# cdglissov/recurrent-flows-msc

Hardware: AMD Instinct MI355X
Metric: frames/sec, RFN SM-MNIST 64x64 train step (fwd+bwd+Adam) (higher is better)
Workload: dtype f32 (forward convolutions fp32-grade: fused scaled-fp16 split f16x3s / three-piece bf16x6 split; gradient convolutions bf16x3 split MFMA; fp32 accumulate everywhere); 1 GPU; RFN SM-MNIST 64x64 canonical (K=10 L=5 Hd=256 h=200 z=56), global_batch=32, seq_len=20, train step; global_batch=32, seq_len=20, parallelism=dp1

## Files before the change

### include/rfn_hip.h

```cpp
#ifndef RFN_HIP_H
#define RFN_HIP_H

#ifdef __cplusplus
extern "C" {
#endif

typedef void* rfn_stream_t;

int rfn_abi_version(void);
const char* rfn_last_error(void);

int rfn_squeeze2d_f32(const float* x, long x_ns, float* y, long y_ns, int N, int C, int H, int W, int undo,
                      rfn_stream_t stream);

int rfn_channel_stats_f32(const float* x, long x_ns, float* mean, float* var_unbiased, int N, int C, int HW,
                          rfn_stream_t stream);

int rfn_actnorm_invconv_fwd_f32(const float* x, long x_ns, const float* bias, const float* logs, const float* Wm,
                                float* z, long z_ns, int N, int C, int HW, rfn_stream_t stream);
int rfn_actnorm_invconv_bwd_f32(const float* x, long x_ns, const float* bias, const float* logs, const float* Wm,
                                const float* gz, long gz_ns, float* gx, long gx_ns, float* gW, float* gbias,
                                float* glogs, int N, int C, int HW, rfn_stream_t stream);
#define RFN_INVCONV_MAX_STEPS 32
#define RFN_INVCONV_MAX_CHANNELS 96
// ... 77 lines not shown
int rfn_gather_affine_f32(const float* P, const float* o_in, long o_ns, const float* b3, const float* l3, float* o_out,
                          float* z, long z_ns, const float* scale, const float* scale_shift, float* logdet,
                          int clamp_type, int N, int C, int H, int W, rfn_stream_t stream);
int rfn_affine_zeros_bwd_f32(const float* zout, long zout_ns, const float* o, long o_ns, const float* gout, long gout_ns,
                             const float* glogdet, const float* scale, const float* scale_shift, const float* l3,
                             float* gz, long gz_ns, float* gpre, long gpre_ns, float* gscale, float* gscale_shift,
                             float* gb3, float* gl3, int clamp_type, int N, int C, int HW, rfn_stream_t stream);

int rfn_glow_shell_fwd_f32(float* z, long z_ns, const float* P, const float* o_in, long o_ns, const float* b3,
                           const float* l3, float* o_out, const float* scale, const float* scale_shift, float* logdet,
                           int clamp_type, const float* bias, const float* logs, const float* Wm, float* znext,
                           long znext_ns, int ld_const, int N, int C, int H, int W, rfn_stream_t stream);
long rfn_glow_shell_fwd_ld_floats(int N, int C, int H, int W);
int rfn_logdet_reduce_f32(const float* part, int n_launch, float* logdet, int accumulate, int N, int C, int H, int W,
                          rfn_stream_t stream);
const char* rfn_glow_shell_fwd_kernel_label(int N, int C, int H, int W, int head);
const char* rfn_glow_shell_bwd_kernel_label(int N, int C, int HW, int tail);
int rfn_glow_shell_supported(int N, int C, int H, int W);
int rfn_glow_shell_bwd_f32(const float* x, long x_ns, const float* bias, const float* logs, const float* Wm,
                           const float* gz, long gz_ns, float* gW, float* gbias, float* glogs, const float* o, long o_ns,
                           const float* glogdet, const float* scale, const float* scale_shift, const float* l3,
                           float* gz_prev, long gz_prev_ns, float* gpre, long gpre_ns, float* gscale,
                           float* gscale_shift, float* gb3, float* gl3, int clamp_type, int ld_const, int N, int C,
                           int HW, rfn_stream_t stream);
int rfn_actnorm_invconv_bwd_ld_f32(const float* x, long x_ns, const float* bias, const float* logs, const float* Wm,
                                   const float* gz, long gz_ns, float* gx, long gx_ns, float* gW, float* gbias,
                                   float* glogs, const float* glogdet, int N, int C, int HW, rfn_stream_t stream);

int rfn_dgrad_small_supported(int N, int Cin, int Cout, int H, int W);
int rfn_conv3x3_smallcout_bf16x3(const float* in, long in_ns, int Cin, const float* wpk, float* out1, long out1_ns,
                                 float* out2, long out2_ns, int Cout, int cout_split, int acc1, int acc2, int N, int H,
                                 int W, rfn_stream_t stream);

int rfn_gemm_wgrad_bf16x3(const float* a, long a_ns, int M, const float* b, long b_ns, int Nc, float* gw, int F, int HW,
                          rfn_stream_t stream);
int rfn_gemm_wgrad_grouped_bf16x3(const float* const* a, long a_ns, int M, const float* const* b, long b_ns, int Nc,
                                  float* const* gw, int G, int F, int HW, rfn_stream_t stream);
const char* rfn_gemm_wgrad_kernel_label_bf16x3(int M, int Nc, long a_ns, long b_ns, int G, int F, int HW);
int rfn_conv3x3_wgrad_implicit_bf16x3(const float* g, long g_ns, int Cout, const float* in1, long in1_ns, int C1,
                                      const float* in2, long in2_ns, int C2, float* gw, int F, int H, int W,
                                      rfn_stream_t stream);
int rfn_conv3x3_wgrad_implicit_grouped_bf16x3(const float* const* g, long g_ns, int Cout, const float* const* in1,
                                              long in1_ns, int C1, const float* const* in2, long in2_ns, int C2,
                                              float* const* gw, int G, int F, int H, int W, rfn_stream_t stream);
const char* rfn_conv3x3_wgrad_implicit_kernel_label_bf16x3(int Cout, long g_ns, int G, int F, int H, int W);
int rfn_im2col3x3_f32(const float* in1, long in1_ns, int C1, const float* in2, long in2_ns, int C2, float* out, int N,
                      int H, int W, rfn_stream_t stream);

long rfn_packed_weight_size(int Cout, int Cin, int ks);
int rfn_pack_conv_weight_f32(const float* w, float* wpk, int Cout, int Cin, int ks, int transpose_flip,
                             rfn_stream_t stream);

int rfn_conv2d_wgrad_f32(const float* in1, long in1_ns, int C1, const float* in2, long in2_ns, int C2,
                         const float* g, long g_ns, int Cout, float* gwt, int N, int H, int W, int ks,
                         rfn_stream_t stream);
const char* rfn_conv2d_wgrad_kernel_label_f32(int ks, int Cin, int Cout, int H, int W);
int rfn_wgrad_finish_f32(const float* gwt, float* gw, int Cout, int Cin, int ks, int accumulate, rfn_stream_t stream);

int rfn_tap_gather_f32(const float* P, const float* bias, const float* logs, float* o, int N, int C, int H, int W,
                       rfn_stream_t stream);
int rfn_tap_scatter_f32(const float* g, float* Gs, int N, int C, int H, int W, rfn_stream_t stream);

int rfn_conv_epilogue_bwd_f32(const float* y, long y_ns, const float* gy, long gy_ns, float* gu, long gu_ns,
                              const float* logs, float* gb, float* gl, int N, int C, int HW, int ep_mode, int act,
                              rfn_stream_t stream);

// ... 127 lines not shown
```

### recurrent-flows-msc_amd/csrc/conv_bf16x3.hip

```cpp
#include "conv_common.h"

typedef __bf16 bf16x8 __attribute__((ext_vector_type(8)));
typedef unsigned int u32x4 __attribute__((ext_vector_type(4)));

static inline void packed_dims_b3(int Cout_l, int Cin_l, int* CoutP, int* Cin16) {
    *CoutP = ((Cout_l + 255) / 256) * 256;
    *Cin16 = (Cin_l + 15) / 16;
}

extern "C" long rfn_packed_weight_size_bf16x3(int Cout, int Cin, int ks) {
    int a, b, c, d;
    packed_dims_b3(Cout, Cin, &a, &b);
    packed_dims_b3(Cin, Cout, &c, &d);
    long s0 = (long)b * ks * ks * 4 * a * 4, s1 = (long)d * ks * ks * 4 * c * 4;
    return s0 > s1 ? s0 : s1;
}
extern "C" long rfn_packed_weight_size_bf16x6(int Cout, int Cin, int ks) {
    return rfn_packed_weight_size_bf16x3(Cout, Cin, ks) / 2 * 3;
}

struct PackDesc {
    const float* w;
    float* wpk;
    int Cout, Cin, ks, mode;
// ... 355 lines not shown
    constexpr int NPOS = (KS == 1) ? 1 : (BPX >= 256 ? 4 : (BPX >= 128 ? 2 : 1));
    constexpr int P2 = (KS == 1 && BPX < 256) ? (BPX >= 64 ? BPX : 64) : 256;
    if (IMG > P2 * NPOS) {
        rfn_set_error("conv2d(bf16x3): map %dx%d needs %d LDS slots (> %d supported)", p.H, p.W, IMG, P2 * NPOS);
        return -7;
    }
    size_t lds = (size_t)NPL * (KC / 8) * IMG * 16 + (size_t)(KC / 16) * KS * KS * NPL * 2 * BCO * 16 + 4 * BCO * 4;
    auto kern = conv_b3_kernel<KS, WCO, WPX, TCO, TPX, KC, NPL>;
    if (lds > 65536) (void)hipFuncSetAttribute((const void*)kern, hipFuncAttributeMaxDynamicSharedMemorySize, (int)lds);
    dim3 grid(p.n_wtiles * p.n_htiles * p.n_ftiles, ceil_div(p.Cout, BCO));
    p.ksplit = 1;
    const int wgs = grid.x * grid.y;
    const int nchunks = (p.Cin8 * 16 + KC - 1) / KC;
    const int HW = p.H * p.W;
    const bool dense = p.out1_ns == (long)p.cout_split * HW &&
                       (p.cout_split == p.Cout || p.out2_ns == (long)(p.Cout - p.cout_split) * HW);
    if (wgs < 128 && nchunks >= 8 && p.ep_mode != 1 && p.ep_mode != 4 && !p.acc1 && !p.acc2 && dense) {
        int ks_ = 512 / wgs;
        if (ks_ > nchunks / 2) ks_ = nchunks / 2;
        if (ks_ > 1) {
            p.ksplit = ks_;
            p.ws_stride = (long)p.N * p.Cout * HW;
            p.ws = rfn_workspace(s, (size_t)ks_ * (size_t)p.ws_stride);
            if (!p.ws) return -8;
        }
    }
    grid.z = p.ksplit;
    hipLaunchKernelGGL(kern, grid, dim3(256), lds, s, p);
    if (p.ksplit > 1) splitk_reduce(p, s);
    return 0;
}

enum ConvB3Route { G3_32x128, G3_64x64, G3_64x128, G1_32x128, G1_64x64, G1_128x128, G1_256x64, WS1, WS3_ACTBWD, WS3_27,
                   WS3_45 };
static const struct { const char* label; int BPX, WPX; } kConvB3Routes[] = {
    {"conv_b3_kernel<3,1,4,1,1,16>", 128, 4},
    {"conv_b3_kernel<3,2,2,1,1,16>", 64, 2},
    {"conv_b3_kernel<3,2,2,1,2,16>", 128, 2},
    {"conv_b3_kernel<1,1,4,1,1,32>", 128, 4},
    {"conv_b3_kernel<1,2,2,1,1,32>", 64, 2},
    {"conv_b3_kernel<1,2,2,2,2,32>", 128, 2},
    {"conv_b3_kernel<1,4,1,2,2,32>", 64, 1},
    {"conv1x1_ws_kernel<16>", 32, 0},
    {"conv3x3_ws_kernel<1,2,0>", 64, 0},
    {"conv3x3_ws_kernel<3,2,1>", 64, 0},
    {"conv3x3_ws_kernel<5,1,1>", 32, 0},
};
static_assert(sizeof(kConvB3Routes) / sizeof(kConvB3Routes[0]) == WS3_45 + 1, "one row per route");

static ConvB3Route choose_conv_b3(const ConvParams& p, int ks) {
    static const bool ws_off = getenv("RFN_CONV_WS") && atoi(getenv("RFN_CONV_WS")) == 0;
    const int Cin = p.C1 + p.C2, Cout = p.Cout;
    const long npix = (long)p.N * p.H * p.W;
    if (p.npl != 3 && !ws_off && Cout % 256 == 0 && npix >= 64L * 256) {
        if (ks == 1 && p.C2 == 0 && Cin > 128 && Cin <= 256) return WS1;
        const int PT = (p.ep_mode == 4 || Cin <= 24) ? 2 : 1;
        const int TH = 32 * PT / (p.W >= 32 ? 32 : (p.W > 0 ? p.W : 1));
        const bool pow2 = (p.H & (p.H - 1)) == 0 && (p.W & (p.W - 1)) == 0;
        if (ks == 3 && pow2 && p.W >= 8 && (long)p.H * p.W >= 64 && p.H >= TH && p.cout_split == Cout && !p.acc1) {
            if (p.ep_mode == 4 && Cin <= 8 && p.C2 == 0) return WS3_ACTBWD;
            if (p.ep_mode >= 0 && p.ep_mode <= 3 && Cin <= 40) return Cin <= 24 ? WS3_27 : WS3_45;
        }
    }
    const bool few_px = npix * ((Cout + 127) / 128) < 256L * 128;
    if (ks == 3) return Cout <= 32 ? G3_32x128 : (few_px ? G3_64x64 : G3_64x128);
    if (Cout <= 32) return G1_32x128;
    if (few_px || Cout <= 64) return G1_64x64;
    return Cout <= 128 ? G1_128x128 : G1_256x64;
}
static int dispatch_conv_b3(ConvParams& p, int ks, hipStream_t s);

static ConvParams conv_b3_shape(int npl, int C1, int C2, int Cout, int cout_split, int acc1, int ep_mode, int N, int H,
                                int W) {
    ConvParams p;
    memset(&p, 0, sizeof(p));
    p.npl = npl; p.C1 = C1; p.C2 = C2; p.Cout = Cout; p.cout_split = cout_split; p.acc1 = acc1; p.ep_mode = ep_mode;
    p.N = N; p.H = H; p.W = W;
    return p;
}
extern "C" const char* rfn_conv2d_kernel_label_bf16x3(int npl, int ks, int C1, int C2, int Cout, int cout_split, int acc1,
                                                     int ep_mode, int N, int H, int W) {
    return kConvB3Routes[choose_conv_b3(conv_b3_shape(npl, C1, C2, Cout, cout_split, acc1, ep_mode, N, H, W), ks)].label;
}
extern "C" int rfn_conv2d_dgrad_act_rows_bf16x3(int N, int H, int W, int ks, int Cout, int Cin) {
    const auto& r = kConvB3Routes[choose_conv_b3(conv_b3_shape(2, Cin, 0, Cout, Cout, 0, 4, N, H, W), ks)];
    if (r.WPX == 0) {
// ... 359 lines not shown
static int launch_conv1x1_ws(ConvParams& p, hipStream_t s) {
    const int HW = p.H * p.W;
    const long total = (long)p.N * HW;
    const int n_tiles = (int)((total + 31) / 32);
    int hw_shift = -1;
    if ((HW & (HW - 1)) == 0) hw_shift = ilog2(HW);
    p.ksplit = 1;
    const size_t lds = (size_t)2 * 2 * 32 * 32 * 16 + 4 * 256 * 4;
    auto kern = conv1x1_ws_kernel<16>;
    (void)hipFuncSetAttribute((const void*)kern, hipFuncAttributeMaxDynamicSharedMemorySize, (int)lds);
    dim3 grid(n_tiles < 256 ? n_tiles : 256, p.Cout / 256);
    hipLaunchKernelGGL(kern, grid, dim3(512), lds, s, p, n_tiles, hw_shift);
    return 0;
}

template <int KS, int WCO, int WPX, int TCO, int TPX, int KC>
static int launch_conv_b3_npl(ConvParams& p, hipStream_t s) {
    return p.npl == 3 ? launch_conv_b3<KS, WCO, WPX, TCO, TPX, KC, 3>(p, s) : launch_conv_b3<KS, WCO, WPX, TCO, TPX, KC>(p, s);
}

static int dispatch_conv_b3(ConvParams& p, int ks, hipStream_t s) {
    switch (choose_conv_b3(p, ks)) {
        case G3_32x128:  return launch_conv_b3_npl<3, 1, 4, 1, 1, 16>(p, s);
        case G3_64x64:   return launch_conv_b3_npl<3, 2, 2, 1, 1, 16>(p, s);
        case G3_64x128:  return launch_conv_b3_npl<3, 2, 2, 1, 2, 16>(p, s);
        case G1_32x128:  return launch_conv_b3_npl<1, 1, 4, 1, 1, 32>(p, s);
        case G1_64x64:   return launch_conv_b3_npl<1, 2, 2, 1, 1, 32>(p, s);
        case G1_128x128: return launch_conv_b3_npl<1, 2, 2, 2, 2, 32>(p, s);
        case G1_256x64:  return launch_conv_b3_npl<1, 4, 1, 2, 2, 32>(p, s);
        case WS1:        return launch_conv1x1_ws(p, s);
        case WS3_ACTBWD: return launch_conv3x3_ws_t<1, 2, false>(p, s);
        case WS3_27:     return launch_conv3x3_ws_t<3, 2>(p, s);
        case WS3_45:     return launch_conv3x3_ws_t<5, 1>(p, s);
    }
    return -9;
}
```

### recurrent-flows-msc_amd/csrc/conv_common.h

```cpp
#pragma once
#include "common.h"
#include "../../include/rfn_hip.h"
#include <stdlib.h>

typedef float f32x16 __attribute__((ext_vector_type(16)));
typedef float f32x4 __attribute__((ext_vector_type(4)));

struct ConvParams {
    const float* in1;
    const float* in2;
    long in1_ns, in2_ns;
    int C1, C2;
    const float* wpk;
    float* out1;
    float* out2;
    long out1_ns, out2_ns;
    int Cout, cout_split, acc1, acc2;
    int N, H, W;
    int CoutP, Cin8;
    int ep_mode, act;
    const float* p0;
    const float* p1;
    int TWp, TH, TF, tw_shift, th_shift;
    int n_wtiles, n_htiles, n_ftiles;
    int P2, P2_shift;
    int ksplit;
    int w_lds_off;
    const float* ybuf;
    long ybuf_ns;
    int npl;
    float* part;
    float* ws;
    long ws_stride;
};

static __global__ void splitk_reduce_kernel(const float* __restrict__ ws, long stride, int ksplit, float* __restrict__ out1,
                                            long n1, float* __restrict__ out2, long n2) {
    const long n = n1 + n2;
    for (long i = (long)blockIdx.x * blockDim.x + threadIdx.x; i < n; i += (long)gridDim.x * blockDim.x) {
        float a = ws[i];
        for (int z = 1; z < ksplit; ++z) a += ws[(long)z * stride + i];
        if (i < n1) out1[i] = a;
        else out2[i - n1] = a;
    }
}
static inline void splitk_reduce(const ConvParams& p, hipStream_t s) {
    const long HW = (long)p.H * p.W, n1 = (long)p.N * p.cout_split * HW, n2 = (long)p.N * (p.Cout - p.cout_split) * HW;
    long blocks = (n1 + n2 + 255) / 256;
    if (blocks > 2048) blocks = 2048;
    hipLaunchKernelGGL(splitk_reduce_kernel, dim3((unsigned)blocks), dim3(256), 0, s, p.ws, p.ws_stride, p.ksplit, p.out1, n1,
                       p.out2, n2);
}

template <int TCO, int TPX, int BCO, bool FASTONLY = false>
__device__ __forceinline__ void conv_epilogue(const ConvParams& p, f32x16 (&acc)[TCO][TPX], const float* ep,
                                              const int co_base, const int wco, const int kk, const int HW,
                                              const int (&pn)[TPX], const int (&ppix)[TPX],
                                              const bool (&pvalid)[TPX], const int prow = 0,
                                              float* const lds_part = nullptr, const bool lds_shared = false) {
    const int cl_base = wco * (32 * TCO) + 4 * kk;
    const bool fast = FASTONLY || ((co_base + 32 * TCO <= p.Cout) && (p.cout_split == p.Cout));
    if (!FASTONLY && p.ep_mode == 4) {
        if (co_base + 32 * TCO > p.Cout) return;
        const float* ybase[TPX];
        float* obase[TPX];
#pragma unroll
        for (int t = 0; t < TPX; ++t) {
            const long off = (long)(co_base + 4 * kk) * HW + ppix[t];
            ybase[t] = pvalid[t] ? p.ybuf + pn[t] * p.ybuf_ns + off : p.ybuf + (long)(co_base + 4 * kk) * HW;
            obase[t] = p.out1 + pn[t] * p.out1_ns + off;
        }
        const int l31 = threadIdx.x & 31;
#pragma unroll
        for (int a = 0; a < TCO; ++a) {
            float yv[16][TPX];
#pragma unroll
            for (int r = 0; r < 16; ++r)
#pragma unroll
                for (int t = 0; t < TPX; ++t)
                    yv[r][t] = ybase[t][(long)(a * 32 + (r & 3) + 8 * (r >> 2)) * HW];
#pragma unroll
            for (int r = 0; r < 16; ++r) {
                const int cidx = a * 32 + (r & 3) + 8 * (r >> 2);
                const float e1 = ep[BCO + cl_base + cidx];
                float sb = 0.f, sl = 0.f;
#pragma unroll
                for (int t = 0; t < TPX; ++t) {
// ... 9 lines not shown
                }
                sb = half_wave_sum_dpp(sb);
                sl = half_wave_sum_dpp(sl);
                if (l31 == 16) {
                    if (lds_part && lds_shared) {
                        float* dst = lds_part + (cl_base + cidx) * 2;
                        atomicAdd(dst, sb);
                        atomicAdd(dst + 1, sl);
                    } else if (lds_part) {
                        float* dst = lds_part + (cl_base + cidx) * 2;
                        dst[0] += sb;
                        dst[1] += sl;
                    } else {
                        float* dst = p.part + co_base + cidx + 4 * kk;
                        atomicAdd(dst, sb);
                        atomicAdd(dst + p.Cout, sl);
                    }
                }
            }
        }
        return;
    }
    if (fast) {
        float* obase[TPX];
        float* const o1 = (!FASTONLY && p.ksplit > 1) ? p.ws + (long)blockIdx.z * p.ws_stride : p.out1;
#pragma unroll
        for (int t = 0; t < TPX; ++t)
            obase[t] = o1 + pn[t] * p.out1_ns + (long)(co_base + 4 * kk) * HW + ppix[t];
#pragma unroll
        for (int a = 0; a < TCO; ++a) {
#pragma unroll
            for (int r = 0; r < 16; ++r) {
                const int cidx = a * 32 + (r & 3) + 8 * (r >> 2);
                float e0 = 0.f, e1 = 1.f;
                if (p.ep_mode != 0) {
                    e0 = blockIdx.z == 0 ? ep[cl_base + cidx] : 0.f;
                    e1 = ep[BCO + cl_base + cidx];
                }
#pragma unroll
                for (int t = 0; t < TPX; ++t) {
                    float v = acc[a][t][r];
                    if (p.ep_mode != 0) v = (v + e0) * e1;
                    if (p.ep_mode == 1) {
                        if (p.act == 1) v = v > 0.f ? v : 0.f;
                        if (p.act == 2) v = v > 0.f ? v : 0.2f * v;
                    }
                    if (pvalid[t]) {
                        float* dst = obase[t] + (long)cidx * HW;
                        if (FASTONLY || p.ksplit > 1) {
                            *dst = v;
                        } else {
                            if (p.acc1) v += *dst;
                            *dst = v;
                        }
                    }
                }
            }
        }
        return;
    }
    if (FASTONLY) return;
#pragma unroll
    for (int a = 0; a < TCO; ++a) {
#pragma unroll
        for (int r = 0; r < 16; ++r) {
            const int cidx = a * 32 + (r & 3) + 8 * (r >> 2);
// ... 12 lines not shown
            const int oc = first ? co : co - p.cout_split;
            const int accm = first ? p.acc1 : p.acc2;
#pragma unroll
            for (int t = 0; t < TPX; ++t) {
                if (!pvalid[t]) continue;
                float v = acc[a][t][r];
                if (p.ep_mode != 0) v = (v + e0) * e1;
                if (p.ep_mode == 1) {
                    if (p.act == 1) v = v > 0.f ? v : 0.f;
                    if (p.act == 2) v = v > 0.f ? v : 0.2f * v;
                }
                float* dst = obase + pn[t] * ons + (long)oc * HW + ppix[t];
                if (p.ksplit > 1) {
                    *dst = v;
                } else {
                    if (accm) v += *dst;
                    *dst = v;
                }
            }
        }
    }
}

static inline void tile_geometry(int H, int W, int BPX, int* TWp, int* TH, int* TF) {
    int tw = next_pow2(W);
    if (tw > 32) tw = 32;
    if (tw > BPX) tw = BPX;
    int th = next_pow2(H);
    if (th > BPX / tw) th = BPX / tw;
    *TWp = tw;
    *TH = th;
    *TF = BPX / (tw * th);
}
```

### recurrent-flows-msc_amd/rfn_hip/lib.py

```python
import ctypes
import os

import torch

_HERE = os.path.dirname(os.path.abspath(__file__))
LIB_PATH = os.path.join(_HERE, "librfn_hip.so")

_c_f = ctypes.c_void_p
_c_i = ctypes.c_int
_c_l = ctypes.c_long
_c_s = ctypes.c_void_p

SIGNATURES = {
    "rfn_abi_version": [],
    "rfn_last_error": [],
    "rfn_squeeze2d_f32": [_c_f, _c_l, _c_f, _c_l, _c_i, _c_i, _c_i, _c_i, _c_i, _c_s],
    "rfn_channel_stats_f32": [_c_f, _c_l, _c_f, _c_f, _c_i, _c_i, _c_i, _c_s],
    "rfn_actnorm_invconv_fwd_f32": [_c_f, _c_l, _c_f, _c_f, _c_f, _c_f, _c_l, _c_i, _c_i, _c_i, _c_s],
    "rfn_actnorm_invconv_bwd_f32": [_c_f, _c_l, _c_f, _c_f, _c_f, _c_f, _c_l, _c_f, _c_l, _c_f, _c_f, _c_f,
                                    _c_i, _c_i, _c_i, _c_s],
    "rfn_invconv_weights_fwd_f32": [ctypes.c_void_p] * 5 + [_c_f, _c_f, _c_i, _c_i, _c_i, _c_s],
    "rfn_invconv_weights_bwd_f32": [ctypes.c_void_p] * 5 + [_c_f, _c_f, _c_f, _c_f, _c_f, _c_i, _c_i, _c_i, _c_s],
    "rfn_invconv_actnorm_rev_f32": [_c_f, _c_l, _c_f, _c_f, _c_f, _c_f, _c_l, _c_i, _c_i, _c_i, _c_s],
    "rfn_conv2d_fwd_f32": [_c_f, _c_l, _c_i, _c_f, _c_l, _c_i, _c_f, _c_f, _c_l, _c_f, _c_l, _c_i, _c_i, _c_i, _c_i,
                           _c_i, _c_i, _c_i, _c_i, _c_i, _c_f, _c_f, _c_i, _c_s],
    "rfn_conv2d_kernel_label_f32": [_c_i] * 5,
    "rfn_conv2d_fwd_bf16x3": [_c_f, _c_l, _c_i, _c_f, _c_l, _c_i, _c_f, _c_f, _c_l, _c_f, _c_l, _c_i, _c_i, _c_i, _c_i,
                              _c_i, _c_i, _c_i, _c_i, _c_i, _c_f, _c_f, _c_i, _c_s],
    "rfn_packed_weight_size_bf16x3": [_c_i, _c_i, _c_i],
    "rfn_pack_conv_weight_bf16x3": [_c_f, _c_f, _c_i, _c_i, _c_i, _c_i, _c_s],
    "rfn_packed_weight_size_bf16x6": [_c_i, _c_i, _c_i],
    "rfn_pack_conv_weight_bf16x6": [_c_f, _c_f, _c_i, _c_i, _c_i, _c_i, _c_s],
    "rfn_conv2d_fwd_bf16x6": [_c_f, _c_l, _c_i, _c_f, _c_l, _c_i, _c_f, _c_f, _c_l, _c_f, _c_l, _c_i, _c_i, _c_i, _c_i,
                              _c_i, _c_i, _c_i, _c_i, _c_i, _c_f, _c_f, _c_i, _c_s],
    "rfn_conv2d_kernel_label_bf16x3": [_c_i] * 11,
    "rfn_conv2d_dgrad_act_rows_bf16x3": [_c_i, _c_i, _c_i, _c_i, _c_i, _c_i],
    "rfn_conv2d_dgrad_act_bf16x3": [_c_f, _c_l, _c_i, _c_f, _c_f, _c_l, _c_f, _c_i, _c_f, _c_l, _c_f, _c_i, _c_i, _c_i,
                                    _c_i, _c_i, _c_s],
    "rfn_gather_affine_f32": [_c_f, _c_f, _c_l, _c_f, _c_f, _c_f, _c_f, _c_l, _c_f, _c_f, _c_f, _c_i, _c_i, _c_i, _c_i,
                              _c_i, _c_s],
    "rfn_affine_zeros_bwd_f32": [_c_f, _c_l, _c_f, _c_l, _c_f, _c_l, _c_f, _c_f, _c_f, _c_f, _c_f, _c_l, _c_f, _c_l, _c_f,
                                 _c_f, _c_f, _c_f, _c_i, _c_i, _c_i, _c_i, _c_s],
    "rfn_glow_shell_fwd_f32": [_c_f, _c_l, _c_f, _c_f, _c_l, _c_f, _c_f, _c_f, _c_f, _c_f, _c_f, _c_i, _c_f, _c_f, _c_f,
                               _c_f, _c_l, _c_i, _c_i, _c_i, _c_i, _c_i, _c_s],
    "rfn_glow_shell_bwd_f32": [_c_f, _c_l, _c_f, _c_f, _c_f, _c_f, _c_l, _c_f, _c_f, _c_f, _c_f, _c_l, _c_f, _c_f, _c_f,
                               _c_f, _c_f, _c_l, _c_f, _c_l, _c_f, _c_f, _c_f, _c_f, _c_i, _c_i, _c_i, _c_i, _c_i, _c_s],
    "rfn_actnorm_invconv_bwd_ld_f32": [_c_f, _c_l, _c_f, _c_f, _c_f, _c_f, _c_l, _c_f, _c_l, _c_f, _c_f, _c_f, _c_f, _c_i,
                                       _c_i, _c_i, _c_s],
    "rfn_dgrad_small_supported": [_c_i, _c_i, _c_i, _c_i, _c_i],
    "rfn_conv3x3_smallcout_bf16x3": [_c_f, _c_l, _c_i, _c_f, _c_f, _c_l, _c_f, _c_l, _c_i, _c_i, _c_i, _c_i, _c_i, _c_i,
                                     _c_i, _c_s],
    "rfn_gemm_wgrad_grouped_bf16x3": [_c_f, _c_l, _c_i, _c_f, _c_l, _c_i, _c_f, _c_i, _c_i, _c_i, _c_s],
    "rfn_conv3x3_wgrad_implicit_grouped_bf16x3": [_c_f, _c_l, _c_i, _c_f, _c_l, _c_i, _c_f, _c_l, _c_i, _c_f, _c_i, _c_i,
                                                  _c_i, _c_i, _c_s],
    "rfn_coupling_po_supported": [_c_i, _c_i, _c_i, _c_i, _c_i, _c_i],
    "rfn_coupling_po_packed_bytes": [_c_i, _c_i],
    "rfn_coupling_po_pack": [_c_f, _c_i, _c_s],
    "rfn_coupling_po_fwd": [_c_f, _c_l, _c_f, _c_l, _c_f, _c_f, _c_f, _c_f, _c_f, _c_f, _c_l, _c_f, _c_l, _c_f, _c_l,
                            _c_f, _c_f, _c_i, _c_i, _c_i, _c_i, _c_i, _c_i, _c_s],
    "rfn_glow_shell_fwd_ld_floats": [_c_i, _c_i, _c_i, _c_i],
    "rfn_logdet_reduce_f32": [_c_f, _c_i, _c_f, _c_i, _c_i, _c_i, _c_i, _c_i, _c_s],
    "rfn_glow_shell_fwd_kernel_label": [_c_i] * 5,
    "rfn_glow_shell_bwd_kernel_label": [_c_i] * 4,
    "rfn_glow_shell_supported": [_c_i] * 4,
    "rfn_coupling_po_mask_floats": [_c_i, _c_i, _c_i],
    "rfn_coupling_po_bwd_supported": [_c_i, _c_i, _c_i, _c_i],
    "rfn_coupling_po_bwd_packed_bytes": [_c_i],
    "rfn_coupling_po_pack_bwd": [_c_f, _c_i, _c_s],
    "rfn_coupling_po_bwd_part_floats": [_c_i, _c_i, _c_i],
    "rfn_coupling_po_bwd": [_c_f, _c_l, _c_f, _c_f, _c_f, _c_f, _c_f, _c_f, _c_l, _c_f, _c_l, _c_f, _c_i, _c_i, _c_i, _c_i,
                            _c_i, _c_s],
    "rfn_coupling_po_bwd_finish": [ctypes.c_void_p] * 8 + [_c_i, _c_i, _c_i, _c_s],
    "rfn_gemm_wgrad_bf16x3": [_c_f, _c_l, _c_i, _c_f, _c_l, _c_i, _c_f, _c_i, _c_i, _c_s],
    "rfn_conv3x3_wgrad_implicit_bf16x3": [_c_f, _c_l, _c_i, _c_f, _c_l, _c_i, _c_f, _c_l, _c_i, _c_f, _c_i, _c_i, _c_i,
                                          _c_s],
    "rfn_gemm_wgrad_kernel_label_bf16x3": [_c_i, _c_i, _c_l, _c_l, _c_i, _c_i, _c_i],
    "rfn_conv3x3_wgrad_implicit_kernel_label_bf16x3": [_c_i, _c_l, _c_i, _c_i, _c_i, _c_i],
    "rfn_im2col3x3_f32": [_c_f, _c_l, _c_i, _c_f, _c_l, _c_i, _c_f, _c_i, _c_i, _c_i, _c_s],
    "rfn_packed_weight_size": [_c_i, _c_i, _c_i],
    "rfn_pack_conv_weight_f32": [_c_f, _c_f, _c_i, _c_i, _c_i, _c_i, _c_s],
    "rfn_conv2d_wgrad_f32": [_c_f, _c_l, _c_i, _c_f, _c_l, _c_i, _c_f, _c_l, _c_i, _c_f, _c_i, _c_i, _c_i, _c_i, _c_s],
    "rfn_conv2d_wgrad_kernel_label_f32": [_c_i] * 5,
    "rfn_wgrad_finish_f32": [_c_f, _c_f, _c_i, _c_i, _c_i, _c_i, _c_s],
    "rfn_tap_gather_f32": [_c_f, _c_f, _c_f, _c_f, _c_i, _c_i, _c_i, _c_i, _c_s],
# ... 145 lines not shown
```

### recurrent-flows-msc_amd/rfn_hip/ops.py

```python
import collections
import ctypes
import functools

import torch

from . import lib as L

_i = ctypes.c_int
_l = ctypes.c_long

import os

CONV_PRECISION = os.environ.get("RFN_CONV_PRECISION", "mixed")


def bwd_b3():
    return CONV_PRECISION in ("bf16x3", "mixed")


MIXED_FWD = os.environ.get("RFN_MIXED_FWD", "bf16x6")


def fwd_prec(H, W):
    if CONV_PRECISION == "mixed":
# ... 309 lines not shown
            assert t[4].numel() == 65536 and t[5].numel() == 65536 and t[2].is_contiguous() and t[5].is_contiguous()
        L.call("rfn_coupling_po_bwd_finish", *cols, _i(len(tk)), _i(nblk), _i(K1),
               meta=_shell("po_bwd_finish", tk[0][7], len(tk) * (nblk * 512 + 512 * K1 + 131072 + 1024) / 1024.0))


def conv2d_raw(in1, in2, wpk, Cout, ks, ep_mode=0, p0=None, p1=None, act=0, out1=None, out2=None, cout_split=None,
               acc1=False, acc2=False, prec=None):
    N, C1, H, W = in1.shape
    C2 = 0 if in2 is None else int(in2.shape[1])
    i1p, i1ns = L.frames(in1, "in1")
    i2p, i2ns = (None, 0) if in2 is None else L.frames(in2, "in2")
    if cout_split is None:
        cout_split = Cout
    if out1 is None:
        out1 = torch.empty((N, cout_split, H, W), device=in1.device, dtype=torch.float32)
    o1p, o1ns = L.frames(out1, "out1")
    o2p, o2ns = (None, 0) if out2 is None else L.frames(out2, "out2")
    prec = prec if prec is not None else ("bf16x3" if bwd_b3() else "f32")
    fn = {"bf16x3": "rfn_conv2d_fwd_bf16x3", "bf16x6": "rfn_conv2d_fwd_bf16x6", "f32": "rfn_conv2d_fwd_f32"}[prec]
    x6 = prec == "bf16x6"
    kname = (kernel_label("rfn_conv2d_kernel_label_f32", ks, Cout, N, H, W) if prec == "f32" else
             kernel_label("rfn_conv2d_kernel_label_bf16x3", 3 if x6 else 2, ks, C1, C2, Cout, cout_split, 1 if acc1 else 0,
                          ep_mode, N, H, W) + (" x6" if x6 else ""))
    L.call(fn, i1p, _l(i1ns), _i(C1), i2p, _l(i2ns), _i(C2),
           L.dev(wpk), o1p, _l(o1ns), o2p,
           _l(o2ns), _i(Cout), _i(cout_split), _i(1 if acc1 else 0), _i(1 if acc2 else 0), _i(N), _i(H), _i(W), _i(ks),
           _i(ep_mode), L.dev(p0), L.dev(p1), _i(act),
           meta=("conv", kname,
                 2.0 * N * H * W * (C1 + C2) * Cout * ks * ks,
                 "N%d %d+%d->%d %dx%d k%d ep%d%s" % (N, C1, C2, Cout, H, W, ks, ep_mode,
                                                  "" if cout_split == Cout else " split"),
                 4.0 * (N * H * W * (C1 + C2 + Cout) + (C1 + C2) * Cout * ks * ks)))
    return out1


def gemm_wgrad(a, b, M, Nc, arena=None):
    F_, HW = int(a.shape[0]), _hw(a)
    ap, ans = L.frames(a, "a")
    bp, bns = L.frames(b, "b")
    gw = _zeros(arena, M, Nc, device=a.device)
    L.call("rfn_gemm_wgrad_bf16x3", ap, _l(ans), _i(M), bp, _l(bns), _i(Nc), L.dev(gw), _i(F_), _i(HW),
           meta=("wgrad", kernel_label("rfn_gemm_wgrad_kernel_label_bf16x3", M, Nc, ans, bns, 0, F_, HW),
                 2.0 * F_ * HW * M * Nc, "F%d %dx%d HW%d" % (F_, M, Nc, HW), 4.0 * (F_ * HW * (M + Nc) + M * Nc)))
    return gw


def conv2d_wgrad_b3(in1, in2, g, Cout, ks, arena=None):
    N, C1, H, W = in1.shape
    C2 = 0 if in2 is None else int(in2.shape[1])
    Cin = C1 + C2
    if ks == 1:
        x = in1 if in2 is None else torch.cat((in1, in2), 1)
        return gemm_wgrad(g, x, Cout, Cin, arena).view(Cout, Cin, 1, 1)
    if Cin <= Cout and W % 8 == 0 and os.environ.get("RFN_WGRAD_IMPLICIT") != "0":
        i1p, i1ns = L.frames(in1, "in1")
        i2p, i2ns = (None, 0) if in2 is None else L.frames(in2, "in2")
        gp, gns = L.frames(g, "g")
        gw = _zeros(arena, Cout, 9 * Cin, device=in1.device)
        L.call("rfn_conv3x3_wgrad_implicit_bf16x3", gp, _l(gns), _i(Cout), i1p, _l(i1ns), _i(C1), i2p, _l(i2ns), _i(C2),
               L.dev(gw), _i(N), _i(H), _i(W),
               meta=("wgrad", kernel_label("rfn_conv3x3_wgrad_implicit_kernel_label_bf16x3", Cout, gns, 0, N, H, W),
                     2.0 * N * H * W * Cout * 9 * Cin, "F%d %dx%d HW%d implicit3x3" % (N, Cout, 9 * Cin, H * W),
                     4.0 * (N * H * W * (Cout + Cin) + Cout * 9 * Cin)))
        return gw.view(Cout, Cin, 3, 3)
    if Cin <= Cout:
        i1p, i1ns = L.frames(in1, "in1")
# ... 1301 lines not shown
```

Before: 11030 frames/s.

## Add persistent register-weight conv3x3 kernel for few-channel convolutions

Adds a new conv3x3 kernel for layers with few input and output channels (at most two 16x32 MFMA tiles). It keeps all weights in registers and runs as a persistent grid over spatial tiles, with a double-buffered LDS halo tile that is split into bf16 planes on the fly. The conv router picks it automatically for qualifying large-pixel convolutions, and an environment variable can turn it off. The aim is to fix poor utilisation and weight-reload overhead of the generic routes on low-channel convolutions, at the cost of heavy register use and one more code path.

```diff
diff --git a/include/rfn_hip.h b/include/rfn_hip.h
--- a/include/rfn_hip.h
+++ b/include/rfn_hip.h
@@ -133,6 +133,12 @@
                                  float* out2, long out2_ns, int Cout, int cout_split, int acc1, int acc2, int N, int H,
                                  int W, rfn_stream_t stream);
 
+int rfn_conv3x3_fewch_supported(int npl, int C1, int C2, int Cout, int H, int W);
+int rfn_conv3x3_fewch_bf16x3(const float* in1, long in1_ns, int C1, const float* in2, long in2_ns, int C2,
+                             const float* wpk, float* out, long out_ns, int Cout, int N, int H, int W, int ep_mode,
+                             const float* p0, const float* p1, int act, int npl, int pt, int max_wgs,
+                             rfn_stream_t stream);
+
 int rfn_gemm_wgrad_bf16x3(const float* a, long a_ns, int M, const float* b, long b_ns, int Nc, float* gw, int F, int HW,
                           rfn_stream_t stream);
 int rfn_gemm_wgrad_grouped_bf16x3(const float* const* a, long a_ns, int M, const float* const* b, long b_ns, int Nc,
diff --git a/recurrent-flows-msc_amd/csrc/conv_bf16x3.hip b/recurrent-flows-msc_amd/csrc/conv_bf16x3.hip
--- a/recurrent-flows-msc_amd/csrc/conv_bf16x3.hip
+++ b/recurrent-flows-msc_amd/csrc/conv_bf16x3.hip
@@ -411,7 +411,7 @@
 }
 
 enum ConvB3Route { G3_32x128, G3_64x64, G3_64x128, G1_32x128, G1_64x64, G1_128x128, G1_256x64, WS1, WS3_ACTBWD, WS3_27,
-                   WS3_45 };
+                   WS3_45, FC3 };
 static const struct { const char* label; int BPX, WPX; } kConvB3Routes[] = {
     {"conv_b3_kernel<3,1,4,1,1,16>", 128, 4},
     {"conv_b3_kernel<3,2,2,1,1,16>", 64, 2},
@@ -424,13 +424,19 @@
     {"conv3x3_ws_kernel<1,2,0>", 64, 0},
     {"conv3x3_ws_kernel<3,2,1>", 64, 0},
     {"conv3x3_ws_kernel<5,1,1>", 32, 0},
+    {"conv3x3_fc_kernel", 256, 0},
 };
-static_assert(sizeof(kConvB3Routes) / sizeof(kConvB3Routes[0]) == WS3_45 + 1, "one row per route");
+static_assert(sizeof(kConvB3Routes) / sizeof(kConvB3Routes[0]) == FC3 + 1, "one row per route");
 
 static ConvB3Route choose_conv_b3(const ConvParams& p, int ks) {
     static const bool ws_off = getenv("RFN_CONV_WS") && atoi(getenv("RFN_CONV_WS")) == 0;
     const int Cin = p.C1 + p.C2, Cout = p.Cout;
     const long npix = (long)p.N * p.H * p.W;
+    static const bool fc_off = getenv("RFN_CONV_FEWCH") && atoi(getenv("RFN_CONV_FEWCH")) == 0;
+    const long fc_min = p.npl == 3 && Cin > 16 ? 524288 : 131072;
+    if (!fc_off && ks == 3 && npix >= fc_min && !(p.npl == 3 && Cout > 32) &&
+        conv3x3_fc_scope(p.C1, p.C2, Cout, p.H, p.W) && p.cout_split == Cout && !p.acc1 && p.ep_mode >= 0 && p.ep_mode <= 2)
+        return FC3;
     if (p.npl != 3 && !ws_off && Cout % 256 == 0 && npix >= 64L * 256) {
         if (ks == 1 && p.C2 == 0 && Cin > 128 && Cin <= 256) return WS1;
         const int PT = (p.ep_mode == 4 || Cin <= 24) ? 2 : 1;
@@ -856,6 +862,7 @@
         case WS3_ACTBWD: return launch_conv3x3_ws_t<1, 2, false>(p, s);
         case WS3_27:     return launch_conv3x3_ws_t<3, 2>(p, s);
         case WS3_45:     return launch_conv3x3_ws_t<5, 1>(p, s);
+        case FC3:        return launch_conv3x3_fc(p, s, 0, 0);
     }
     return -9;
 }
diff --git a/recurrent-flows-msc_amd/csrc/conv_common.h b/recurrent-flows-msc_amd/csrc/conv_common.h
--- a/recurrent-flows-msc_amd/csrc/conv_common.h
+++ b/recurrent-flows-msc_amd/csrc/conv_common.h
@@ -52,7 +52,7 @@
                        p.out2, n2);
 }
 
-template <int TCO, int TPX, int BCO, bool FASTONLY = false>
+template <int TCO, int TPX, int BCO, bool FASTONLY = false, bool RAGGED8 = false>
 __device__ __forceinline__ void conv_epilogue(const ConvParams& p, f32x16 (&acc)[TCO][TPX], const float* ep,
                                               const int co_base, const int wco, const int kk, const int HW,
                                               const int (&pn)[TPX], const int (&ppix)[TPX],
@@ -128,6 +128,7 @@
 #pragma unroll
             for (int r = 0; r < 16; ++r) {
                 const int cidx = a * 32 + (r & 3) + 8 * (r >> 2);
+                if (RAGGED8 && co_base + cidx >= p.Cout) continue;
                 float e0 = 0.f, e1 = 1.f;
                 if (p.ep_mode != 0) {
                     e0 = blockIdx.z == 0 ? ep[cl_base + cidx] : 0.f;
@@ -206,3 +207,6 @@
     *TH = th;
     *TF = BPX / (tw * th);
 }
+
+bool conv3x3_fc_scope(int C1, int C2, int Cout, int H, int W);
+int launch_conv3x3_fc(ConvParams& p, hipStream_t s, int pt, int max_wgs);
diff --git a/recurrent-flows-msc_amd/csrc/conv_fewch.hip b/recurrent-flows-msc_amd/csrc/conv_fewch.hip
--- /dev/null
+++ b/recurrent-flows-msc_amd/csrc/conv_fewch.hip
@@ -0,0 +1,246 @@
+#include "conv_common.h"
+
+typedef __bf16 bf16x8 __attribute__((ext_vector_type(8)));
+
+template <int C16, int TCO, int PT, int NPL, int OCC>
+__global__ __launch_bounds__(256, OCC) void conv3x3_fc_kernel(const ConvParams p, const int n_tiles, const int tw_shift,
+                                                              const int tpf_shift, const int wt_shift) {
+    constexpr int NG = 2 * C16, NK = 9 * C16, BCO = 32 * TCO;
+    constexpr int IMGP = PT == 2 ? 340 : 204;
+    constexpr int NPOS = (IMGP + 255) / 256;
+    extern __shared__ __attribute__((aligned(16))) unsigned char lds_raw[];
+    const int TW = 1 << tw_shift, TH = (128 * PT) >> tw_shift;
+    const int IMGW = TW + 2, IMG = IMGW * (TH + 2);
+    bf16x8* Bs = reinterpret_cast<bf16x8*>(lds_raw);
+    float* ep = reinterpret_cast<float*>(Bs + 2 * NPL * NG * IMGP);
+    const int tid = threadIdx.x, lane = tid & 63;
+    const int wave = __builtin_amdgcn_readfirstlane(tid >> 6);
+    const int l31 = lane & 31, kk = lane >> 5;
+    const int HW = p.H * p.W, Cin = p.C1 + p.C2;
+
+    bf16x8 wr[TCO][NK][NPL];
+    {
+        const bf16x8* wp = reinterpret_cast<const bf16x8*>(p.wpk) + l31;
+#pragma unroll
+        for (int s = 0; s < NK; ++s) {
+            const int tap = s / C16, c16 = s % C16;
+#pragma unroll
+            for (int pl = 0; pl < NPL; ++pl)
+#pragma unroll
+                for (int a = 0; a < TCO; ++a)
+                    wr[a][s][pl] = wp[(long)(((c16 * 9 + tap) * NPL + pl) * 2 + kk) * p.CoutP + a * 32];
+        }
+    }
+    if (p.ep_mode != 0) {
+        for (int c = tid; c < BCO; c += 256) {
+            float e0 = 0.f, e1 = 1.f;
+            if (c < p.Cout) {
+                e0 = p.p0[c];
+                if (p.ep_mode == 1) e1 = expf(p.p1[c]);
+                if (p.ep_mode == 2) e1 = expf(3.f * p.p1[c]);
+            }
+            ep[c] = e0;
+            ep[BCO + c] = e1;
+        }
+    }
+
+    int srel[NPOS], syx[NPOS];
+#pragma unroll
+    for (int j = 0; j < NPOS; ++j) {
+        const int pos = tid + 256 * j;
+        const int syy = pos / IMGW, sxx = pos - syy * IMGW;
+        srel[j] = syy * p.W + sxx;
+        syx[j] = pos < IMG ? (syy << 16) | sxx : -1;
+    }
+    float stg[NG][NPOS][8];
+    unsigned sok = 0;
+    auto tile_origin = [&](int tile, int& n, int& y0, int& x0) {
+        n = tile >> tpf_shift;
+        const int r = tile & ((1 << tpf_shift) - 1);
+        y0 = (r >> wt_shift) * TH;
+        x0 = (r & ((1 << wt_shift) - 1)) * TW;
+    };
+    auto prefetch = [&](int tile) {
+        const bool tv = tile < n_tiles;
+        int n, y0, x0;
+        tile_origin(tv ? tile : 0, n, y0, x0);
+        const long corner = (long)(y0 - 1) * p.W + x0 - 1;
+        const long b1 = (long)n * p.in1_ns + corner, b2 = (long)n * p.in2_ns + corner;
+        unsigned rel[NPOS];
+        sok = 0;
+#pragma unroll
+        for (int j = 0; j < NPOS; ++j) {
+            const int gy = y0 + (syx[j] >> 16) - 1, gx = x0 + (syx[j] & 0xFFFF) - 1;
+            const bool ok = tv && syx[j] >= 0 && (unsigned)gy < (unsigned)p.H && (unsigned)gx < (unsigned)p.W;
+            sok |= ok ? 1u << j : 0u;
+            rel[j] = ok ? srel[j] : p.W + 1;
+        }
+#pragma unroll
+        for (int g = 0; g < NG; ++g)
+#pragma unroll
+            for (int c = 0; c < 8; ++c) {
+                const int ch = g * 8 + c < Cin ? g * 8 + c : 0;
+                const float* src = ch < p.C1 ? p.in1 + (b1 + (long)ch * HW) : p.in2 + (b2 + (long)(ch - p.C1) * HW);
+#pragma unroll
+                for (int j = 0; j < NPOS; ++j) stg[g][j][c] = src[rel[j]];
+            }
+    };
+    auto commit = [&](int buf) {
+        bf16x8* dst = Bs + buf * (NPL * NG * IMGP) + tid;
+#pragma unroll
+        for (int j = 0; j < NPOS; ++j) {
+            if (syx[j] < 0) continue;
+            const bool ok = (sok >> j) & 1u;
+#pragma unroll
+            for (int g = 0; g < NG; ++g) {
+                bf16x8 hi, lo, l3;
+#pragma unroll
+                for (int c = 0; c < 8; ++c) {
+                    const float v = (ok && g * 8 + c < Cin) ? stg[g][j][c] : 0.f;
+                    const __bf16 h = (__bf16)v;
+                    const float r1 = v - (float)h;
+                    const __bf16 m = (__bf16)r1;
+                    hi[c] = h;
+                    lo[c] = m;
+                    if (NPL == 3) l3[c] = (__bf16)(r1 - (float)m);
+                }
+                dst[(0 * NG + g) * IMGP + 256 * j] = hi;
+                dst[(1 * NG + g) * IMGP + 256 * j] = lo;
+                if (NPL == 3) dst[(2 * NG + g) * IMGP + 256 * j] = l3;
+            }
+        }
+    };
+
+    int pcol[PT], prow[PT], pbase[PT][3];
+#pragma unroll
+    for (int t = 0; t < PT; ++t) {
+        const int px = (wave * PT + t) * 32 + l31;
+        pcol[t] = px & (TW - 1);
+        prow[t] = px >> tw_shift;
+#pragma unroll
+        for (int dy = 0; dy < 3; ++dy) pbase[t][dy] = (prow[t] + dy) * IMGW + pcol[t] + kk * IMGP;
+    }
+    int tile = blockIdx.x, buf = 0;
+    prefetch(tile);
+    for (; tile < n_tiles; tile += gridDim.x, buf ^= 1) {
+        commit(buf);
+        prefetch(tile + gridDim.x);
+        __builtin_amdgcn_sched_barrier(0);
+        __syncthreads();
+        const bf16x8* bb = Bs + buf * (NPL * NG * IMGP);
+        f32x16 acc[TCO][PT];
+#pragma unroll
+        for (int a = 0; a < TCO; ++a)
+#pragma unroll
+            for (int t = 0; t < PT; ++t)
+#pragma unroll
+                for (int r = 0; r < 16; ++r) acc[a][t][r] = 0.f;
+#pragma unroll
+        for (int s = 0; s < NK; ++s) {
+            const int tap = s / C16, c16 = s % C16;
+            const int off = 2 * c16 * IMGP + tap % 3;
+            bf16x8 b[PT][NPL];
+#pragma unroll
+            for (int t = 0; t < PT; ++t)
+#pragma unroll
+                for (int pl = 0; pl < NPL; ++pl) b[t][pl] = bb[pl * NG * IMGP + pbase[t][tap / 3] + off];
+            constexpr int NPR = NPL == 3 ? 6 : 3;
+            constexpr int PA[6] = {1, 0, NPL == 3 ? 2 : 0, 0, 1, 0};
+            constexpr int PB[6] = {NPL == 3 ? 1 : 0, NPL == 3 ? 2 : 1, 0, 1, 0, 0};
+#pragma unroll
+            for (int q = 0; q < NPR; ++q)
+#pragma unroll
+                for (int a = 0; a < TCO; ++a)
+#pragma unroll
+                    for (int t = 0; t < PT; ++t)
+                        acc[a][t] = __builtin_amdgcn_mfma_f32_32x32x16_bf16(wr[a][s][PA[q]], b[t][PB[q]], acc[a][t], 0, 0, 0);
+        }
+        int n, y0, x0;
+        tile_origin(tile, n, y0, x0);
+        int pn[PT], ppix[PT];
+        bool pvalid[PT];
+#pragma unroll
+        for (int t = 0; t < PT; ++t) {
+            pn[t] = n;
+            ppix[t] = (y0 + prow[t]) * p.W + x0 + pcol[t];
+            pvalid[t] = true;
+        }
+        conv_epilogue<TCO, PT, BCO, true, true>(p, acc, ep, 0, 0, kk, HW, pn, ppix, pvalid);
+    }
+}
+
+bool conv3x3_fc_scope(int C1, int C2, int Cout, int H, int W) {
+    if (C1 <= 0 || C2 < 0 || Cout <= 0 || (Cout & 7) || H < 16 || W < 16) return false;
+    if ((H & (H - 1)) || (W & (W - 1)) || (long)H * W > (1L << 20)) return false;
+    return ((C1 + C2 + 15) / 16) * ((Cout + 31) / 32) <= 2;
+}
+
+template <int C16, int TCO, int PT, int NPL, int OCC>
+static int launch_fc_t(ConvParams& p, hipStream_t s, int max_wgs) {
+    const int TW = p.W < 32 ? p.W : 32, TH = 128 * PT / TW;
+    const int tw_shift = ilog2(TW);
+    const int wt = p.W / TW, ht = p.H / TH;
+    const int wt_shift = ilog2(wt), tpf_shift = ilog2(wt * ht);
+    const long n_tiles = (long)p.N * wt * ht;
+    constexpr int IMGP = PT == 2 ? 340 : 204;
+    const int IMG = (TW + 2) * (TH + 2);
+    if (IMG > IMGP || n_tiles > 0x7FFFFFFFL - 65536) {
+        rfn_set_error("conv3x3_fc: %d image positions, %ld tiles", IMG, n_tiles);
+        return -8;
+    }
+    const size_t lds = (size_t)2 * NPL * 2 * C16 * IMGP * 16 + 2 * 32 * TCO * 4;
+    auto kern = conv3x3_fc_kernel<C16, TCO, PT, NPL, OCC>;
+    if (lds > 65536) (void)hipFuncSetAttribute((const void*)kern, hipFuncAttributeMaxDynamicSharedMemorySize, (int)lds);
+    const int cap = max_wgs > 0 ? max_wgs : 256 * OCC;
+    hipLaunchKernelGGL(kern, dim3((unsigned)(n_tiles < cap ? n_tiles : cap)), dim3(256), lds, s, p, (int)n_tiles, tw_shift,
+                       tpf_shift, wt_shift);
+    return 0;
+}
+
+template <int PT, int NPL>
+static int launch_fc_shape(ConvParams& p, hipStream_t s, int max_wgs) {
+    const bool rows2 = p.Cout > 32, k2 = p.C1 + p.C2 > 16;
+    if (NPL == 3) {
+        if (rows2) return launch_fc_t<1, 2, 1, 3, 1>(p, s, max_wgs);
+        if (k2) return launch_fc_t<2, 1, PT, 3, 1>(p, s, max_wgs);
+        return launch_fc_t<1, 1, PT, 3, 2>(p, s, max_wgs);
+    }
+    if (rows2) return launch_fc_t<1, 2, 1, 2, 2>(p, s, max_wgs);
+    if (k2) return launch_fc_t<2, 1, 1, 2, 2>(p, s, max_wgs);
+    return launch_fc_t<1, 1, PT, 2, 2>(p, s, max_wgs);
+}
+
+int launch_conv3x3_fc(ConvParams& p, hipStream_t s, int pt, int max_wgs) {
+    p.ksplit = 1;
+    if (pt == 0) pt = (long)p.N * p.H * p.W >= 2048L * 256 ? 2 : 1;
+    if (p.npl == 3) return pt == 2 ? launch_fc_shape<2, 3>(p, s, max_wgs) : launch_fc_shape<1, 3>(p, s, max_wgs);
+    return pt == 2 ? launch_fc_shape<2, 2>(p, s, max_wgs) : launch_fc_shape<1, 2>(p, s, max_wgs);
+}
+
+extern "C" int rfn_conv3x3_fewch_supported(int npl, int C1, int C2, int Cout, int H, int W) {
+    return (npl == 2 || npl == 3) && conv3x3_fc_scope(C1, C2, Cout, H, W) ? 1 : 0;
+}
+
+extern "C" int rfn_conv3x3_fewch_bf16x3(const float* in1, long in1_ns, int C1, const float* in2, long in2_ns, int C2,
+                                        const float* wpk, float* out, long out_ns, int Cout, int N, int H, int W,
+                                        int ep_mode, const float* p0, const float* p1, int act, int npl, int pt,
+                                        int max_wgs, rfn_stream_t stream) {
+    RFN_CHECK_ARG(in1 && wpk && out && N >= 0 && (C2 == 0 || in2), -1);
+    RFN_CHECK_ARG(rfn_conv3x3_fewch_supported(npl, C1, C2, Cout, H, W), -2);
+    RFN_CHECK_ARG(ep_mode >= 0 && ep_mode <= 2 && (ep_mode == 0 || (p0 && p1)), -3);
+    RFN_CHECK_ARG(((uintptr_t)wpk & 15) == 0 && pt >= 0 && pt <= 2 && max_wgs >= 0, -4);
+    RFN_CHECK_ARG(in1_ns >= (long)C1 * H * W && (C2 == 0 || in2_ns >= (long)C2 * H * W) && out_ns >= (long)Cout * H * W, -5);
+    if (N == 0) return 0;
+    ConvParams p;
+    memset(&p, 0, sizeof(p));
+    p.in1 = in1; p.in2 = in2; p.in1_ns = in1_ns; p.in2_ns = in2_ns; p.C1 = C1; p.C2 = C2;
+    p.wpk = wpk; p.out1 = out; p.out1_ns = out_ns; p.Cout = Cout; p.cout_split = Cout;
+    p.N = N; p.H = H; p.W = W;
+    p.CoutP = ((Cout + 255) / 256) * 256;
+    p.Cin8 = (C1 + C2 + 15) / 16;
+    p.ep_mode = ep_mode; p.act = act; p.p0 = p0; p.p1 = p1; p.npl = npl;
+    int rc = launch_conv3x3_fc(p, (hipStream_t)stream, pt, max_wgs);
+    if (rc) return rc;
+    RFN_LAUNCH_CHECK();
+    return 0;
+}
diff --git a/recurrent-flows-msc_amd/rfn_hip/lib.py b/recurrent-flows-msc_amd/rfn_hip/lib.py
--- a/recurrent-flows-msc_amd/rfn_hip/lib.py
+++ b/recurrent-flows-msc_amd/rfn_hip/lib.py
@@ -50,6 +50,9 @@
     "rfn_dgrad_small_supported": [_c_i, _c_i, _c_i, _c_i, _c_i],
     "rfn_conv3x3_smallcout_bf16x3": [_c_f, _c_l, _c_i, _c_f, _c_f, _c_l, _c_f, _c_l, _c_i, _c_i, _c_i, _c_i, _c_i, _c_i,
                                      _c_i, _c_s],
+    "rfn_conv3x3_fewch_supported": [_c_i] * 6,
+    "rfn_conv3x3_fewch_bf16x3": [_c_f, _c_l, _c_i, _c_f, _c_l, _c_i, _c_f, _c_f, _c_l, _c_i, _c_i, _c_i, _c_i, _c_i, _c_f,
+                                 _c_f, _c_i, _c_i, _c_i, _c_i, _c_s],
     "rfn_gemm_wgrad_grouped_bf16x3": [_c_f, _c_l, _c_i, _c_f, _c_l, _c_i, _c_f, _c_i, _c_i, _c_i, _c_s],
     "rfn_conv3x3_wgrad_implicit_grouped_bf16x3": [_c_f, _c_l, _c_i, _c_f, _c_l, _c_i, _c_f, _c_l, _c_i, _c_f, _c_i, _c_i,
                                                   _c_i, _c_i, _c_s],
diff --git a/recurrent-flows-msc_amd/rfn_hip/ops.py b/recurrent-flows-msc_amd/rfn_hip/ops.py
--- a/recurrent-flows-msc_amd/rfn_hip/ops.py
+++ b/recurrent-flows-msc_amd/rfn_hip/ops.py
@@ -365,6 +365,28 @@
                                                   "" if cout_split == Cout else " split"),
                  4.0 * (N * H * W * (C1 + C2 + Cout) + (C1 + C2) * Cout * ks * ks)))
     return out1
+
+
+def conv3x3_fewch_ok(prec, C1, C2, Cout, H, W):
+    return prec in ("bf16x3", "bf16x6") and bool(L.load().rfn_conv3x3_fewch_supported(
+        3 if prec == "bf16x6" else 2, int(C1), int(C2), int(Cout), int(H), int(W)))
+
+
+def conv3x3_fewch(in1, in2, wpk, Cout, prec="bf16x3", ep_mode=0, p0=None, p1=None, act=0, out=None, pt=0, max_wgs=0):
+    N, C1, H, W = in1.shape
+    C2 = 0 if in2 is None else int(in2.shape[1])
+    i1p, i1ns = L.frames(in1, "in1")
+    i2p, i2ns = (None, 0) if in2 is None else L.frames(in2, "in2")
+    if out is None:
+        out = torch.empty((N, Cout, H, W), device=in1.device, dtype=torch.float32)
+    op, ons = L.frames(out, "out")
+    x6 = prec == "bf16x6"
+    L.call("rfn_conv3x3_fewch_bf16x3", i1p, _l(i1ns), _i(C1), i2p, _l(i2ns), _i(C2), L.dev(wpk), op, _l(ons), _i(Cout),
+           _i(N), _i(H), _i(W), _i(ep_mode), L.dev(p0), L.dev(p1), _i(act), _i(3 if x6 else 2), _i(pt), _i(max_wgs),
+           meta=("conv", "conv3x3_fc_kernel" + (" x6" if x6 else ""), 2.0 * N * H * W * (C1 + C2) * Cout * 9,
+                 "N%d %d+%d->%d %dx%d k3 ep%d" % (N, C1, C2, Cout, H, W, ep_mode),
+                 4.0 * (N * H * W * (C1 + C2 + Cout) + (C1 + C2) * Cout * 9)))
+    return out
 
 
 def gemm_wgrad(a, b, M, Nc, arena=None):
```

Measured after the change: 11140 frames/s, median of 6. Within noise of the previous version (+1.0%).
